# SGI-2022/Latent-Diffusion-Models-for-Shape-SDFs

Hardware: AMD Instinct MI355X
Metric: SDF queries/sec on 256^3 grid (+ DDPM sample steps/sec) (higher is better)
Workload: dtype bf16; 1 GPU; config4: decode B=64 shapes on a 256^3 grid on 1 rank (the whole grid is the one slab: no gather); batch=64, grid=256, latent_dim=256, decoder=DeepSDF 8x512 skip@4, parallelism=zslab1

## Files before the change

latent-diffusion-models-for-shape-sdfs_amd/csrc/decoder_fs.hip:

```cpp
#include "decoder_common.h"

namespace ldm {
namespace {
using namespace dec;

constexpr int kFsD = 4;
constexpr int kFsDefaultV = 2;

constexpr int kFsStep = 2048;
constexpr int kFsAct = 33 * 4 * 1024;
constexpr int kFsRed = 4 * 4 * 64 * 4;
constexpr int kFsWl = 512 * 4;
#ifndef FS_STAMP
#define FS_STAMP 0
#endif
constexpr int kFsStamp = FS_STAMP ? 128 * 8 : 0;
#ifndef FS_ABL
#define FS_ABL 0
#endif
static_assert(FS_ABL == 0 || FS_STAMP, "ablations are diagnostic builds");
constexpr int kFsLds = kFsAct + kFsRed + kFsWl + kFsStamp;
static_assert(kFsLds <= 160 * 1024, "LDS");

__host__ __device__ constexpr int fs_nparts(int S) { return S == 256 ? 15 : 16; }
__host__ __device__ constexpr int fs_nsteps(int S) { return S == 256 ? 384 : 448; }

template <typename T>
__global__ void fs_aux_pack_kernel(const float* __restrict__ beta, const float* __restrict__ wxyz,
                                   int B, T* __restrict__ aux) {
    const int id = blockIdx.x * blockDim.x + threadIdx.x;
    if (id >= B * 4 * 4 * 2 * 64) return;
    const int lane = id & 63;
    const int i = (id >> 6) & 1;
    const int slot = (id >> 7) & 3;
    const int w = (id >> 9) & 3;
    const int b = id >> 11;
    const int li = slot >> 1;
    const int p = slot & 1;
    float v[8] = {0, 0, 0, 0, 0, 0, 0, 0};
    if (lane < 32) {
        const int f = 128 * w + 64 * p + 32 * i + lane;
        const float* wx = wxyz + ((size_t)li * kHidden + f) * 3;
        const float bb = beta[((size_t)b * 2 + li) * kHidden + f];
        const float hi = Elem<T>::round(bb);
        v[0] = wx[0]; v[1] = wx[1]; v[2] = wx[2];
        v[3] = wx[0]; v[4] = wx[1]; v[5] = wx[2];
        v[6] = hi;    v[7] = bb - hi;
    }
    T* o = aux + (size_t)id * 8;
#pragma unroll
    for (int e = 0; e < 8; ++e) o[e] = (T)v[e];
}

struct FArgs {
    const uint8_t* stream;
    const uint8_t* aux;
    const float* w_last;
    const float* xyz;
    float* out;
    float b_last;
    int npts, tiles_per_shape, n_tiles;
    int N, k0;
    float vs, origin;
};

enum FsEpi { FE_NONE = 0, FE_LATE = 1, FE_EARLY = 2, FE_FIN0 = 3, FE_FIN1 = 4 };

struct FSrc {
    bool shape;
    uint32_t off;
    bool none = false;
};

template <int FV>
struct FCtx {
    int lane, wave, h;
    uint32_t voff;
    char* smem;
    __amdgpu_buffer_rsrc_t rw;
    __amdgpu_buffer_rsrc_t ra;
    uint32_t s_beg, s_end;
    uint32_t s_iss;
    uint32_t baux_w;
    uint32_t aux_w;
    uint32_t aux_next;
    u32x4 auxn[2];
    u32x4 ring[kFsD][2];
    u32x4 b[4];
    float part[4];
    float* out;
    int npts, prev_shape, prev_local;
    float b_last;
    unsigned long long* st;
    int st_i;
    bool st_on;
};

template <int FV>
__device__ __forceinline__ void stamp(FCtx<FV>& c) {
    if (FS_STAMP) {
        if (c.st_on && c.lane == 0 && c.st_i < 128) c.st[c.st_i] = __builtin_readcyclecounter();
        ++c.st_i;
    }
}

__device__ __forceinline__ u32x4 bld(__amdgpu_buffer_rsrc_t r, uint32_t voff, uint32_t soff) {
    return __builtin_bit_cast(u32x4, __builtin_amdgcn_raw_buffer_load_b128(r, voff, soff, 0));
}

template <int FV>
__device__ __forceinline__ void load_aux(FCtx<FV>& c, FSrc s) {
    if (s.none) return;
    const __amdgpu_buffer_rsrc_t r = s.shape ? c.ra : c.rw;
    c.auxn[0] = bld(r, c.voff, s.off);
    c.auxn[1] = bld(r, c.voff + 1024u, s.off);
}

__device__ __forceinline__ uint32_t opaque(uint32_t v) {
    asm volatile("" : "+v"(v));
    return v;
}

__device__ __forceinline__ int opaque_s(int v) {
    asm volatile("" : "+s"(v));
    return v;
}

template <int FV>
__device__ __forceinline__ char* lds_at(const FCtx<FV>& c, uint32_t off) {
    return c.smem + (opaque(c.voff) + off);
}
template <int FV>
__device__ __forceinline__ u32x4* act_w(const FCtx<FV>& c, int late) {
    return reinterpret_cast<u32x4*>(lds_at(c, (uint32_t)(late + 4 * c.wave) * 4096u));
}
template <int FV>
__device__ __forceinline__ const f32x4* wl_at(const FCtx<FV>& c, int p, int i) {
    const uint32_t h = opaque(c.voff) >> 9;
    return reinterpret_cast<const f32x4*>(
        c.smem + kFsAct + kFsRed + (((c.wave * 2 + p) * 2 + i) * 2) * 64 + h * 64);
}

template <int FV>
__device__ __forceinline__ float* red_w(const FCtx<FV>& c) {
    return reinterpret_cast<float*>(c.smem + kFsAct + c.wave * 4 * 64 * 4 + (opaque(c.voff) >> 2));
}

__device__ __forceinline__ void fs_bar() {
    if (FS_ABL & 4) return;
    asm volatile("s_waitcnt lgkmcnt(0)\n\ts_barrier" ::: "memory");
}

template <int FV>
__device__ __forceinline__ void read_b(FCtx<FV>& c, int pos) {
    const u32x4* p = reinterpret_cast<const u32x4*>(lds_at(c, pos * 4096));
#pragma unroll
    for (int n = 0; n < 4; ++n) c.b[n] = p[n * 64];
}

template <int FV>
__device__ __forceinline__ void issue(FCtx<FV>& c, int r) {
    const uint32_t so = c.s_iss + (uint32_t)(r >> 1) * 2u * kFsStep;
    const uint32_t vo = c.voff + (uint32_t)(r & 1) * kFsStep;
    if (FS_ABL & 1) return;
    c.ring[r][0] = bld(c.rw, vo, so);
    c.ring[r][1] = bld(c.rw, vo + 1024u, so);
}

template <int FV>
__device__ __forceinline__ void next_group(FCtx<FV>& c) {
    c.s_iss += 4u * kFsStep;
    if (c.s_iss == c.s_end) c.s_iss = c.s_beg;
}

__device__ __forceinline__ float relu_f(float x) {
    return __builtin_bit_cast(float, max(__builtin_bit_cast(int, x), 0));
}

template <typename T, int EK, int FV>
__device__ __forceinline__ void epi_unit(FCtx<FV>& c, const f32x16 (&accY)[2][4], int u) {
    const int t = u >> 1, s = u & 1;
    const int i = t >> 2, n = t & 3;
    if (FS_ABL & 2) return;
    if (EK == FE_LATE || EK == FE_EARLY) {
        u32x4 f;
#pragma unroll
        for (int q = 0; q < 4; ++q)
            f[q] = relu2(Elem<T>::pack(accY[i][n][8 * s + 2 * q], accY[i][n][8 * s + 2 * q + 1]));
        u32x4* p = act_w(c, EK == FE_LATE ? 16 : 0);
        p[((2 * i + s) * 4 + n) * 64] = f;
    } else if (EK == FE_FIN0 || EK == FE_FIN1) {
        const f32x4* w = wl_at(c, EK == FE_FIN0 ? 0 : 1, i);
        float part = c.part[n];
#pragma unroll
        for (int q = 2 * s; q < 2 * s + 2; ++q) {
            const f32x4 wv = w[q];
#pragma unroll
            for (int e = 0; e < 4; ++e) part = fmaf(relu_f(accY[i][n][4 * q + e]), wv[e], part);
        }
        c.part[n] = part;
    }
}

template <typename T, int EK, int FV>
__device__ __forceinline__ void epi_step(FCtx<FV>& c, const f32x16 (&accY)[2][4], int k) {
    if (EK == FE_NONE || k == 15) return;
    epi_unit<T, EK>(c, accY, k);
    if (k == 14) epi_unit<T, EK>(c, accY, 15);
    if (EK == FE_FIN1 && k == 14) {
        float* rw = red_w(c);
#pragma unroll
        for (int n = 0; n < 4; ++n) {
            rw[n * 64] = c.part[n];
            c.part[n] = 0.f;
        }
    }
}

template <int FV>
__device__ __forceinline__ void fin_store(const FCtx<FV>& c, int shape, int local) {
    const int lane = (int)(opaque(c.voff) >> 4);
    if (local < 0 || lane >= 32) return;
    const float* rr = reinterpret_cast<const float*>(
        c.smem + kFsAct + c.wave * 64 * 4 + (opaque(c.voff) >> 2));
    float s = 0.f;
#pragma unroll
    for (int w = 0; w < 4; ++w) s += rr[w * 4 * 64] + rr[w * 4 * 64 + 32];
    const int pt = local * kTilePoints + 32 * c.wave + lane;
    if (pt < c.npts) {
        const __amdgpu_buffer_rsrc_t ro = __builtin_amdgcn_make_buffer_rsrc(
            (void*)(c.out + (size_t)shape * c.npts), (short)0, 0x7ffffff0, 0x00020000);
        __builtin_amdgcn_raw_buffer_store_b32(__builtin_bit_cast(uint32_t, tanhf(s + c.b_last)),
                                              ro, (uint32_t)pt * 4u, 0, 2 );
    }
}

__device__ __forceinline__ void valu_slot(int v) {
    if (v == 2) __builtin_amdgcn_sched_group_barrier(0x002, 2, 0);
    else if (v == 4) __builtin_amdgcn_sched_group_barrier(0x002, 4, 0);
}

template <typename T>
__device__ __forceinline__ void mfma_pair(f32x16 (&acc)[2][4], const u32x4& a0, const u32x4& a1,
                                          const u32x4& b, int n) {
    acc[0][n] = Elem<T>::mfma(a0, b, acc[0][n]);
    acc[1][n] = Elem<T>::mfma(a1, b, acc[1][n]);
}

template <typename T, int EK, int K0, int BAR, int FV>
__device__ __forceinline__ void group4(FCtx<FV>& c, f32x16 (&acc)[2][4], const f32x16 (&accY)[2][4],
                                       int p0) {
    constexpr int BP = (FV & 1) ? 2 : 1;
    const char* gbase = (FV & 2) ? lds_at(c, (p0 + 1) * 4096) : nullptr;
#pragma unroll
    for (int r = 0; r < 4; ++r) {
        const u32x4* nb = reinterpret_cast<const u32x4*>(
            (FV & 2) ? gbase + r * 4096 : lds_at(c, (p0 + r + 1) * 4096));
        const u32x4 a0 = c.ring[r][0], a1 = c.ring[r][1];
        const int k = K0 + r;
        const int V = (EK == FE_NONE || k == 15) ? 0 : (k == 14 ? 4 : 2);
        if (r == BAR) {
#pragma unroll
            for (int n = 0; n < BP; ++n) mfma_pair<T>(acc, a0, a1, c.b[n], n);
            for (int n = 0; n < BP; ++n) {
                __builtin_amdgcn_sched_group_barrier(0x008, 2, 0);
            }
            __builtin_amdgcn_sched_barrier(0);
            fs_bar();
            __builtin_amdgcn_sched_barrier(0);
#pragma unroll
            for (int n = 0; n < BP; ++n) c.b[n] = nb[n * 64];
#pragma unroll
            for (int n = BP; n < 4; ++n) {
                mfma_pair<T>(acc, a0, a1, c.b[n], n);
                c.b[n] = nb[n * 64];
            }
            issue(c, r);
            epi_step<T, EK>(c, accY, k);
            for (int n = 0; n < BP; ++n) __builtin_amdgcn_sched_group_barrier(0x100, 1, 0);
            for (int n = BP; n < 4; ++n) {
                __builtin_amdgcn_sched_group_barrier(0x008, 1, 0);
                valu_slot(V);
                __builtin_amdgcn_sched_group_barrier(0x008, 1, 0);
                __builtin_amdgcn_sched_group_barrier(0x100, 1, 0);
                valu_slot(V);
            }
        } else {
#pragma unroll
            for (int n = 0; n < 4; ++n) {
                mfma_pair<T>(acc, a0, a1, c.b[n], n);
                c.b[n] = nb[n * 64];
            }
            issue(c, r);
            epi_step<T, EK>(c, accY, k);
#pragma unroll
            for (int n = 0; n < 4; ++n) {
                __builtin_amdgcn_sched_group_barrier(0x008, 1, 0);
                valu_slot(V);
                __builtin_amdgcn_sched_group_barrier(0x008, 1, 0);
                __builtin_amdgcn_sched_group_barrier(0x100, 1, 0);
                valu_slot(V);
            }
        }
        __builtin_amdgcn_sched_group_barrier(0x020, 2, 0);
        __builtin_amdgcn_sched_barrier(0);
    }
    next_group(c);
}

template <typename T, int EK, bool BAR, int FV>
__device__ __forceinline__ void steps16e(FCtx<FV>& c, f32x16 (&acc)[2][4],
                                         const f32x16 (&accY)[2][4], int p0) {
    group4<T, EK, 0, -1, FV>(c, acc, accY, p0);
    group4<T, EK, 4, -1, FV>(c, acc, accY, p0 + 4);
    group4<T, EK, 8, -1, FV>(c, acc, accY, p0 + 8);
    group4<T, EK, 12, BAR ? 3 : -1, FV>(c, acc, accY, p0 + 12);
}

template <typename T, int FV>
__device__ __forceinline__ void steps_plain(FCtx<FV>& c, f32x16 (&acc)[2][4],
                                            const f32x16 (&accY)[2][4], int pos0, int j0, int j1) {
#pragma unroll 1
    for (int j = j0; j < j1; j += 4) group4<T, FE_NONE, 0, -1, FV>(c, acc, accY, pos0 + j);
}

template <typename T, int EK, bool E16, int FV>
__device__ __forceinline__ void run_part(FCtx<FV>& c, f32x16 (&acc)[2][4], const f32x16 (&accY)[2][4],
                                         int nk, bool mid, bool endbar, FSrc naux, int pos0,
                                         bool bar0) {
    const f32x16 zero = {};
    const u32x4 a0 = c.auxn[0], a1 = c.auxn[1];
    if (nk == 0) {
#pragma unroll
        for (int n = 0; n < 4; ++n) {
            acc[0][n] = Elem<T>::mfma(a0, c.b[n], zero);
            acc[1][n] = Elem<T>::mfma(a1, c.b[n], zero);
        }
        load_aux(c, naux);
        stamp(c);
        return;
    }
    if (bar0) {
#pragma unroll
        for (int n = 0; n < 4; ++n) {
            acc[0][n] = Elem<T>::mfma(a0, c.b[n], zero);
            acc[1][n] = Elem<T>::mfma(a1, c.b[n], zero);
        }
        load_aux(c, naux);
        fs_bar();
        read_b(c, pos0);
    } else {
        const u32x4* p = reinterpret_cast<const u32x4*>(lds_at(c, pos0 * 4096));
#pragma unroll
        for (int n = 0; n < 4; ++n) {
            acc[0][n] = Elem<T>::mfma(a0, c.b[n], zero);
            acc[1][n] = Elem<T>::mfma(a1, c.b[n], zero);
            c.b[n] = p[n * 64];
        }
        load_aux(c, naux);
#pragma unroll
        for (int n = 0; n < 4; ++n) {
            __builtin_amdgcn_sched_group_barrier(0x008, 2, 0);
            __builtin_amdgcn_sched_group_barrier(0x100, 1, 0);
        }
        __builtin_amdgcn_sched_group_barrier(0x020, 2, 0);
        __builtin_amdgcn_sched_barrier(0);
    }
    stamp(c);
    if (!E16 && EK != FE_NONE) {
        if (mid || (endbar && nk == 16)) steps16e<T, EK, true>(c, acc, accY, pos0);
        else steps16e<T, EK, false>(c, acc, accY, pos0);
        if (EK == FE_FIN1) fin_store(c, c.prev_shape, c.prev_local);
        stamp(c);
        if (endbar && nk == 32) {
            steps_plain<T>(c, acc, accY, pos0, 16, 28);
            group4<T, FE_NONE, 0, 3, FV>(c, acc, accY, pos0 + 28);
        } else {
            steps_plain<T>(c, acc, accY, pos0, 16, nk);
        }
    } else if (E16) {
        steps_plain<T>(c, acc, accY, pos0, 0, 12);
        group4<T, FE_NONE, 0, 3, FV>(c, acc, accY, pos0 + 12);
        stamp(c);
        if (endbar) steps16e<T, EK, true>(c, acc, accY, pos0 + 16);
        else steps16e<T, EK, false>(c, acc, accY, pos0 + 16);
    } else {
        steps_plain<T>(c, acc, accY, pos0, 0, nk < 16 ? nk : 16);
        stamp(c);
        steps_plain<T>(c, acc, accY, pos0, 16, nk);
    }
    stamp(c);
}

template <typename T, bool LATE, int FV>
__device__ __forceinline__ void acc_to_lds(FCtx<FV>& c, const f32x16 (&acc)[2][4]) {
    u32x4* p = act_w(c, LATE ? 16 : 0);
#pragma unroll
    for (int i = 0; i < 2; ++i)
#pragma unroll
        for (int n = 0; n < 4; ++n) {
            u32x4 f0, f1;
            acc_to_frags<T>(acc[i][n], f0, f1);
            p[(2 * i * 4 + n) * 64] = f0;
            p[((2 * i + 1) * 4 + n) * 64] = f1;
        }
}

template <typename T, int S, bool POINTS, int FV>
__global__ __launch_bounds__(256, 1) void dec_fs_kernel(FArgs a) {
    __shared__ __attribute__((aligned(16))) char smem[kFsLds];
    FCtx<FV> c;
    c.lane = threadIdx.x & 63;
    c.wave = __builtin_amdgcn_readfirstlane(threadIdx.x >> 6);
    c.h = c.lane >> 5;
    c.voff = (uint32_t)c.lane * 16u;
    c.smem = smem;
    c.out = a.out;
    c.npts = a.npts;
    c.b_last = a.b_last;
    c.prev_shape = 0;
    c.prev_local = -1;
    c.st = reinterpret_cast<unsigned long long*>(smem + kFsAct + kFsRed + kFsWl);
    c.st_i = 0;
    c.st_on = false;
    float* wl = reinterpret_cast<float*>(smem + kFsAct + kFsRed);

    for (int i = threadIdx.x; i < 512; i += 256) wl[i] = a.w_last[i];
    __syncthreads();
    if ((int)blockIdx.x >= a.n_tiles) return;

    constexpr int NST = fs_nsteps(S);
    constexpr int NP = fs_nparts(S);
    constexpr uint32_t kFlags = 0x00020000u;
    c.rw = __builtin_amdgcn_make_buffer_rsrc((void*)a.stream, (short)0, 0x7ffffff0, kFlags);
    c.ra = __builtin_amdgcn_make_buffer_rsrc((void*)a.aux, (short)0, 0x7ffffff0, kFlags);
    c.s_beg = (uint32_t)c.wave * NST * kFsStep;
    c.s_end = c.s_beg + NST * kFsStep;
    c.s_iss = c.s_beg;
    c.baux_w = (uint32_t)(4 * NST + c.wave * NP) * kFsStep;
    auto shape_aux = [&](int tile) -> uint32_t {
        return ((uint32_t)(tile / a.tiles_per_shape) * 4u + (uint32_t)c.wave) * 4u * kFsStep;
    };
    auto bias = [&](int pi) -> FSrc { return FSrc{false, c.baux_w + (uint32_t)pi * kFsStep}; };
    auto shp = [&](int slot) -> FSrc { return FSrc{true, c.aux_w + (uint32_t)slot * kFsStep}; };
    c.aux_w = shape_aux(blockIdx.x);
#pragma unroll
    for (int r = 0; r < kFsD; ++r) issue(c, r);
    next_group(c);

    f32x16 accA[2][4], accB[2][4];
#pragma unroll
    for (int i = 0; i < 2; ++i)
#pragma unroll
        for (int n = 0; n < 4; ++n) accB[i][n] = f32x16{};
#pragma unroll
    for (int n = 0; n < 4; ++n) c.part[n] = 0.f;
#pragma unroll 1
    for (int tile = blockIdx.x; tile < a.n_tiles; tile += gridDim.x) {
        const int shape = tile / a.tiles_per_shape;
        const int local = tile - shape * a.tiles_per_shape;
        {
            const int nt = tile + (int)gridDim.x;
            c.aux_next = nt < a.n_tiles ? shape_aux(nt) : c.aux_w;
        }
        c.st_on = FS_STAMP && c.wave == 0 && tile == (int)blockIdx.x + (int)gridDim.x;
        c.st_i = 0;
        stamp(c);
        load_aux(c, shp(0));
        const uint32_t lv = opaque(c.voff);
        const bool hi = lv >= 512u;
#pragma unroll
        for (int n = 0; n < 4; ++n) {
            int pt = local * kTilePoints + 32 * n + (int)((lv >> 4) & 31u);
            if (pt >= a.npts) pt = a.npts - 1;
            float x, y, z;
            if (POINTS) {
                const float* qq = a.xyz + ((size_t)shape * a.npts + pt) * 3;
                x = qq[0];
                y = qq[1];
                z = qq[2];
            } else {
                grid_point(pt, opaque_s(a.N), a.k0, a.vs, a.origin, x, y, z);
            }
            const float xh = Elem<T>::round(x), yh = Elem<T>::round(y), zh = Elem<T>::round(z);
            u32x4 f;
            f[0] = hi ? 0u : Elem<T>::pack(xh, yh);
            f[1] = hi ? 0u : Elem<T>::pack(zh, x - xh);
            f[2] = hi ? 0u : Elem<T>::pack(y - yh, z - zh);
            f[3] = hi ? 0u : Elem<T>::pack(1.f, 1.f);
            reinterpret_cast<u32x4*>(lds_at(c, 32u * 4096u))[n * 64] = f;
        }
        read_b(c, 32);

        run_part<T, FE_NONE, false, FV>(c, accA, accB, 0, false, false, shp(1), 0, false);
        acc_to_lds<T, false, FV>(c, accA);
        stamp(c);
        run_part<T, FE_NONE, false, FV>(c, accA, accB, 0, false, false, bias(2), 0, false);
        acc_to_lds<T, true, FV>(c, accA);
        stamp(c);

        int pi = 2;
        run_part<T, FE_FIN1, false, FV>(c, accA, accB, 32, true, false, bias(pi + 1), 0, true);
        run_part<T, FE_EARLY, true, FV>(c, accB, accA, 32, true, true, bias(pi + 2), 0, false);
        pi += 2;
        constexpr int L2P = S == 256 ? 3 : 4;
#pragma unroll 1
        for (int l = 2; l < L2P; ++l, pi += 2) {
            const FSrc nx = (S == 512 && l == 3) ? shp(2) : bias(pi + 2);
            run_part<T, FE_LATE, false, FV>(c, accA, accB, 32, true, false, bias(pi + 1), 0, false);
            run_part<T, FE_EARLY, true, FV>(c, accB, accA, 32, true, true, nx, 0, false);
        }
        if (S == 256) {
            run_part<T, FE_LATE, false, FV>(c, accA, accB, 32, true, false, shp(2), 0, false);
            fs_bar();
            acc_to_lds<T, true, FV>(c, accA);
            stamp(c);
            run_part<T, FE_NONE, false, FV>(c, accA, accB, 16, false, false, shp(3), 16, true);
            run_part<T, FE_EARLY, false, FV>(c, accB, accA, 16, false, true, bias(pi + 3), 16,
                                             false);
            pi += 3;
        } else {
            run_part<T, FE_LATE, false, FV>(c, accA, accB, 32, true, false, shp(3), 0, false);
            run_part<T, FE_EARLY, true, FV>(c, accB, accA, 32, true, true, bias(pi + 2), 0, false);
            pi += 2;
        }
#pragma unroll 1
        for (int l = 5; l < 7; ++l, pi += 2) {
            run_part<T, FE_LATE, false, FV>(c, accA, accB, 32, true, false, bias(pi + 1), 0, false);
            run_part<T, FE_EARLY, true, FV>(c, accB, accA, 32, true, true, bias(pi + 2), 0, false);
        }
        run_part<T, FE_LATE, false, FV>(c, accA, accB, 32, true, false, bias(pi + 1), 0, false);
        run_part<T, FE_FIN0, false, FV>(c, accB, accA, 32, false, true, FSrc{true, 0, true}, 0,
                                        false);
        c.prev_shape = shape;
        c.prev_local = local;
        c.aux_w = c.aux_next;
    }
#pragma unroll
    for (int u = 0; u < 16; ++u) epi_unit<T, FE_FIN1>(c, accB, u);
    {
        float* rw = red_w(c);
#pragma unroll
        for (int n = 0; n < 4; ++n) rw[n * 64] = c.part[n];
    }
    fs_bar();
    fin_store(c, c.prev_shape, c.prev_local);
    asm volatile("s_waitcnt vmcnt(0)" ::: "memory");
    if (FS_STAMP && c.wave == 0) {
        __builtin_amdgcn_s_waitcnt(0);
        for (int k = c.lane; k < 128; k += 64)
            reinterpret_cast<unsigned long long*>(a.out)[(size_t)blockIdx.x * 128 + k] = c.st[k];
    }
}

template <typename T, int S, int D>
void launch_fs_d(const FArgs& a, bool points, hipStream_t s, int grid) {
    if (points)
        hipLaunchKernelGGL((dec_fs_kernel<T, S, true, D>), dim3(grid), dim3(256), 0, s, a);
    else
        hipLaunchKernelGGL((dec_fs_kernel<T, S, false, D>), dim3(grid), dim3(256), 0, s, a);
}

template <typename T, int S>
void launch_fs(const FArgs& a, bool points, hipStream_t s, int grid) {
#ifdef LDM_DEV_KNOBS
    switch (dev_knob("LDM_FS_V", kFsDefaultV)) {
        case 0: return launch_fs_d<T, S, 0>(a, points, s, grid);
        case 1: return launch_fs_d<T, S, 1>(a, points, s, grid);
        case 3: return launch_fs_d<T, S, 3>(a, points, s, grid);
        default: break;
    }
#endif
    launch_fs_d<T, S, kFsDefaultV>(a, points, s, grid);
}

}

size_t decoder_fs_aux_bytes(int B) { return (size_t)B * 4 * 4 * kFsStep; }

int decoder_fs_n_stages(int skip_width) { return fs_nsteps(skip_width == 253 ? 256 : 512); }

int decoder_fs_fwd(const ldm_decoder_t* w, const float* beta, const float* xyz, int B, int npts,
                   int N, int k0, float vs, float origin, float* out, void* ws, size_t ws_bytes,
                   hipStream_t s, int num_cus) {
    const int S = w->skip_width == 253 ? 256 : 512;
    LDM_REQUIRE(w->n_stages == fs_nsteps(S), LDM_EINVAL, "split layout: n_stages %d != %d",
                w->n_stages, fs_nsteps(S));
    LDM_REQUIRE(ws != nullptr && ws_bytes >= decoder_fs_aux_bytes(B) && LDM_ALIGNED(ws, 16),
                LDM_ENOSPC, "workspace too small: need %zu bytes, got %zu",
                decoder_fs_aux_bytes(B), ws_bytes);
    LDM_REQUIRE((size_t)B * 4 * 4 * kFsStep < 0x7ffffff0u, LDM_EINVAL,
                "split layout: %d shapes exceed the aux buffer range", B);
    {
        const int n = B * 4 * 4 * 2 * 64;
        if (w->dtype == LDM_BF16)
            hipLaunchKernelGGL(fs_aux_pack_kernel<__bf16>, dim3((n + 255) / 256), dim3(256), 0, s,
                               beta, w->wxyz, B, (__bf16*)ws);
        else
            hipLaunchKernelGGL(fs_aux_pack_kernel<_Float16>, dim3((n + 255) / 256), dim3(256), 0,
                               s, beta, w->wxyz, B, (_Float16*)ws);
        if (int e = launch_status("fs_aux_pack")) return e;
    }
    FArgs a;
    a.stream = (const uint8_t*)w->weights;
    a.aux = (const uint8_t*)ws;
    a.w_last = w->w_last;
    a.xyz = xyz;
    a.out = out;
    a.b_last = w->b_last;
    a.npts = npts;
    a.tiles_per_shape = (npts + kTilePoints - 1) / kTilePoints;
    a.n_tiles = B * a.tiles_per_shape;
    a.N = N;
    a.k0 = k0;
    a.vs = vs;
    a.origin = origin;
    const int grid = a.n_tiles < num_cus ? a.n_tiles : num_cus;
    const bool points = xyz != nullptr;
    if (w->dtype == LDM_BF16) {
        if (S == 256) launch_fs<__bf16, 256>(a, points, s, grid);
        else launch_fs<__bf16, 512>(a, points, s, grid);
    } else {
        if (S == 256) launch_fs<_Float16, 256>(a, points, s, grid);
        else launch_fs<_Float16, 512>(a, points, s, grid);
    }
    return launch_status("ldm_decoder_fwd(split)");
}

}
```

latent-diffusion-models-for-shape-sdfs_amd/csrc/decoder_common.h:

```cpp
#pragma once
#include "ldm_internal.h"

#include <math.h>

namespace ldm {
namespace dec {

#define LDM_STR2(x) #x
#define LDM_STR(x) LDM_STR2(x)

__device__ __forceinline__ float grid_axis(int i, float vs, float origin) {
#pragma clang fp contract(off)
    float t = (float)i * vs;
    return t + origin;
}

__device__ __forceinline__ void grid_point(int p, int N, int k0, float vs, float origin,
                                           float& x, float& y, float& z) {
    const int nn = N * N;
    const int k = k0 + p / nn;
    const int r = p - (p / nn) * nn;
    const int j = r / N;
    const int i = r - j * N;
    x = grid_axis(i, vs, origin);
    y = grid_axis(j, vs, origin);
    z = grid_axis(k, vs, origin);
}


template <typename T>
struct Elem;
template <>
struct Elem<__bf16> {
    static __device__ __forceinline__ unsigned pack(float a, float b) {
        typedef float f32x2 __attribute__((ext_vector_type(2)));
        const f32x2 v = {a, b};
        return __builtin_bit_cast(unsigned, __builtin_convertvector(v, bf16x2));
    }
    static __device__ __forceinline__ float round(float x) { return (float)(__bf16)x; }
    static __device__ __forceinline__ f32x16 mfma(u32x4 a, u32x4 b, f32x16 c) {
        return __builtin_amdgcn_mfma_f32_32x32x16_bf16(__builtin_bit_cast(bf16x8, a),
                                                       __builtin_bit_cast(bf16x8, b), c, 0, 0, 0);
    }
    static __device__ __forceinline__ f32x4 mfma16(u32x4 a, u32x4 b, f32x4 c) {
        return __builtin_amdgcn_mfma_f32_16x16x32_bf16(__builtin_bit_cast(bf16x8, a),
                                                       __builtin_bit_cast(bf16x8, b), c, 0, 0, 0);
    }
};
template <>
struct Elem<_Float16> {
    static __device__ __forceinline__ unsigned pack(float a, float b) {
        f16x2 v = {(_Float16)a, (_Float16)b};
        return __builtin_bit_cast(unsigned, v);
    }
    static __device__ __forceinline__ float round(float x) { return (float)(_Float16)x; }
    static __device__ __forceinline__ f32x16 mfma(u32x4 a, u32x4 b, f32x16 c) {
        return __builtin_amdgcn_mfma_f32_32x32x16_f16(__builtin_bit_cast(f16x8, a),
                                                      __builtin_bit_cast(f16x8, b), c, 0, 0, 0);
    }
    static __device__ __forceinline__ f32x4 mfma16(u32x4 a, u32x4 b, f32x4 c) {
        return __builtin_amdgcn_mfma_f32_16x16x32_f16(__builtin_bit_cast(f16x8, a),
                                                      __builtin_bit_cast(f16x8, b), c, 0, 0, 0);
    }
};


__device__ __forceinline__ unsigned relu2(unsigned v) {
    typedef short s16x2 __attribute__((ext_vector_type(2)));
    s16x2 x = __builtin_bit_cast(s16x2, v);
    const s16x2 z = {0, 0};
    x = __builtin_elementwise_max(x, z);
    return __builtin_bit_cast(unsigned, x);
}

template <typename T>
__device__ __forceinline__ void acc_to_frags(const f32x16& a, u32x4& f0, u32x4& f1) {
#pragma unroll
    for (int q = 0; q < 4; ++q) {
        f0[q] = relu2(Elem<T>::pack(a[2 * q], a[2 * q + 1]));
        f1[q] = relu2(Elem<T>::pack(a[8 + 2 * q], a[8 + 2 * q + 1]));
    }
}

}
}
```

Before: 469.1 million queries/s.

## Overlap next tile's xyz encoding and first layer with last layer's tail

Moves the computation of the next tile's input coordinates and its first layer MFMAs into the final layer part of the current tile, so the prologue of each tile overlaps the previous tile's epilogue instead of running serially at loop top. Grid-point index decomposition now uses host-precomputed magic-number division instead of integer division. The stamp instrumentation is made branch-free with a dummy slot. This adds register pressure and complexity in the loop-carried state (shape/local handoff).

```diff
diff --git a/latent-diffusion-models-for-shape-sdfs_amd/csrc/decoder_fs.hip b/latent-diffusion-models-for-shape-sdfs_amd/csrc/decoder_fs.hip
--- a/latent-diffusion-models-for-shape-sdfs_amd/csrc/decoder_fs.hip
+++ b/latent-diffusion-models-for-shape-sdfs_amd/csrc/decoder_fs.hip
@@ -14,7 +14,7 @@
 #ifndef FS_STAMP
 #define FS_STAMP 0
 #endif
-constexpr int kFsStamp = FS_STAMP ? 128 * 8 : 0;
+constexpr int kFsStamp = FS_STAMP ? 129 * 8 : 0;
 #ifndef FS_ABL
 #define FS_ABL 0
 #endif
@@ -62,14 +62,25 @@
     int npts, tiles_per_shape, n_tiles;
     int N, k0;
     float vs, origin;
+    uint32_t mN, mNN;
+    int shN, shNN;
 };
+
+inline void fs_magic(uint32_t d, uint32_t& m, int& sh) {
+    int l = 0;
+    while ((1ull << l) < d) ++l;
+    sh = 31 + l;
+    m = (uint32_t)(((1ull << sh) + d - 1) / d);
+}
+__device__ __forceinline__ int fs_div(int n, uint32_t m, int sh) {
+    return (int)(((uint64_t)(uint32_t)n * m) >> sh);
+}
 
 enum FsEpi { FE_NONE = 0, FE_LATE = 1, FE_EARLY = 2, FE_FIN0 = 3, FE_FIN1 = 4 };
 
 struct FSrc {
     bool shape;
     uint32_t off;
-    bool none = false;
 };
 
 template <int FV>
@@ -99,7 +110,7 @@
 template <int FV>
 __device__ __forceinline__ void stamp(FCtx<FV>& c) {
     if (FS_STAMP) {
-        if (c.st_on && c.lane == 0 && c.st_i < 128) c.st[c.st_i] = __builtin_readcyclecounter();
+        c.st[c.st_on && c.st_i < 128 ? c.st_i : 128] = __builtin_readcyclecounter();
         ++c.st_i;
     }
 }
@@ -110,7 +121,6 @@
 
 template <int FV>
 __device__ __forceinline__ void load_aux(FCtx<FV>& c, FSrc s) {
-    if (s.none) return;
     const __amdgpu_buffer_rsrc_t r = s.shape ? c.ra : c.rw;
     c.auxn[0] = bld(r, c.voff, s.off);
     c.auxn[1] = bld(r, c.voff + 1024u, s.off);
@@ -118,11 +128,6 @@
 
 __device__ __forceinline__ uint32_t opaque(uint32_t v) {
     asm volatile("" : "+v"(v));
-    return v;
-}
-
-__device__ __forceinline__ int opaque_s(int v) {
-    asm volatile("" : "+s"(v));
     return v;
 }
 
@@ -370,7 +375,10 @@
     if (!E16 && EK != FE_NONE) {
         if (mid || (endbar && nk == 16)) steps16e<T, EK, true>(c, acc, accY, pos0);
         else steps16e<T, EK, false>(c, acc, accY, pos0);
-        if (EK == FE_FIN1) fin_store(c, c.prev_shape, c.prev_local);
+        if (EK == FE_FIN1) {
+            stamp(c);
+            fin_store(c, c.prev_shape, c.prev_local);
+        }
         stamp(c);
         if (endbar && nk == 32) {
             steps_plain<T>(c, acc, accY, pos0, 16, 28);
@@ -404,6 +412,80 @@
             p[(2 * i * 4 + n) * 64] = f0;
             p[((2 * i + 1) * 4 + n) * 64] = f1;
         }
+}
+
+template <typename T, bool POINTS, int FV>
+__device__ __forceinline__ u32x4 xyz_frag(const FCtx<FV>& c, const FArgs& a, int shape, int local,
+                                          int n) {
+    const uint32_t lv = opaque(c.voff);
+    const bool hi = lv >= 512u;
+    int pt = local * kTilePoints + 32 * n + (int)((lv >> 4) & 31u);
+    if (pt >= a.npts) pt = a.npts - 1;
+    float x, y, z;
+    if (POINTS) {
+        const float* qq = a.xyz + ((size_t)shape * a.npts + pt) * 3;
+        x = qq[0];
+        y = qq[1];
+        z = qq[2];
+    } else {
+        const int k = fs_div(pt, a.mNN, a.shNN);
+        const int r = pt - k * (a.N * a.N);
+        const int j = fs_div(r, a.mN, a.shN);
+        x = grid_axis(r - j * a.N, a.vs, a.origin);
+        y = grid_axis(j, a.vs, a.origin);
+        z = grid_axis(a.k0 + k, a.vs, a.origin);
+    }
+    const float xh = Elem<T>::round(x), yh = Elem<T>::round(y), zh = Elem<T>::round(z);
+    u32x4 f;
+    f[0] = hi ? 0u : Elem<T>::pack(xh, yh);
+    f[1] = hi ? 0u : Elem<T>::pack(zh, x - xh);
+    f[2] = hi ? 0u : Elem<T>::pack(y - yh, z - zh);
+    f[3] = hi ? 0u : Elem<T>::pack(1.f, 1.f);
+    reinterpret_cast<u32x4*>(lds_at(c, 32u * 4096u))[n * 64] = f;
+    return f;
+}
+
+template <typename T, bool POINTS, int FV>
+__device__ __forceinline__ void run_l7p1(FCtx<FV>& c, f32x16 (&acc)[2][4], f32x16 (&accY)[2][4],
+                                         const FArgs& a, int nshape, int nlocal) {
+    const f32x16 zero = {};
+    {
+        const u32x4 a0 = c.auxn[0], a1 = c.auxn[1];
+        const u32x4* p = reinterpret_cast<const u32x4*>(lds_at(c, 0));
+#pragma unroll
+        for (int n = 0; n < 4; ++n) {
+            acc[0][n] = Elem<T>::mfma(a0, c.b[n], zero);
+            acc[1][n] = Elem<T>::mfma(a1, c.b[n], zero);
+            c.b[n] = p[n * 64];
+        }
+        load_aux(c, FSrc{true, c.aux_next});
+#pragma unroll
+        for (int n = 0; n < 4; ++n) {
+            __builtin_amdgcn_sched_group_barrier(0x008, 2, 0);
+            __builtin_amdgcn_sched_group_barrier(0x100, 1, 0);
+        }
+        __builtin_amdgcn_sched_group_barrier(0x020, 2, 0);
+        __builtin_amdgcn_sched_barrier(0);
+    }
+    stamp(c);
+    steps16e<T, FE_FIN0, true>(c, acc, accY, 0);
+    stamp(c);
+#pragma unroll
+    for (int n = 0; n < 4; ++n) {
+        const u32x4 f = xyz_frag<T, POINTS>(c, a, nshape, nlocal, n);
+        if (FS_STAMP) {
+            __builtin_amdgcn_sched_barrier(0);
+            stamp(c);
+        }
+        accY[0][n] = Elem<T>::mfma(c.auxn[0], f, zero);
+        accY[1][n] = Elem<T>::mfma(c.auxn[1], f, zero);
+        __builtin_amdgcn_sched_barrier(0);
+        stamp(c);
+    }
+    load_aux(c, FSrc{true, c.aux_next + (uint32_t)kFsStep});
+    __builtin_amdgcn_sched_barrier(0);
+    steps16e<T, FE_EARLY, true>(c, acc, accY, 16);
+    stamp(c);
 }
 
 template <typename T, int S, bool POINTS, int FV>
@@ -455,45 +537,26 @@
         for (int n = 0; n < 4; ++n) accB[i][n] = f32x16{};
 #pragma unroll
     for (int n = 0; n < 4; ++n) c.part[n] = 0.f;
+    int shape = (int)blockIdx.x / a.tiles_per_shape;
+    int local = (int)blockIdx.x - shape * a.tiles_per_shape;
+    load_aux(c, shp(0));
+#pragma unroll
+    for (int n = 0; n < 4; ++n) c.b[n] = xyz_frag<T, POINTS>(c, a, shape, local, n);
+    run_part<T, FE_NONE, false, FV>(c, accA, accB, 0, false, false, shp(1), 0, false);
+    acc_to_lds<T, false, FV>(c, accA);
 #pragma unroll 1
     for (int tile = blockIdx.x; tile < a.n_tiles; tile += gridDim.x) {
-        const int shape = tile / a.tiles_per_shape;
-        const int local = tile - shape * a.tiles_per_shape;
+        int nshape = shape, nlocal = local;
         {
             const int nt = tile + (int)gridDim.x;
-            c.aux_next = nt < a.n_tiles ? shape_aux(nt) : c.aux_w;
+            if (nt < a.n_tiles) {
+                nshape = nt / a.tiles_per_shape;
+                nlocal = nt - nshape * a.tiles_per_shape;
+            }
+            c.aux_next = ((uint32_t)nshape * 4u + (uint32_t)c.wave) * 4u * kFsStep;
         }
         c.st_on = FS_STAMP && c.wave == 0 && tile == (int)blockIdx.x + (int)gridDim.x;
         c.st_i = 0;
-        stamp(c);
-        load_aux(c, shp(0));
-        const uint32_t lv = opaque(c.voff);
-        const bool hi = lv >= 512u;
-#pragma unroll
-        for (int n = 0; n < 4; ++n) {
-            int pt = local * kTilePoints + 32 * n + (int)((lv >> 4) & 31u);
-            if (pt >= a.npts) pt = a.npts - 1;
-            float x, y, z;
-            if (POINTS) {
-                const float* qq = a.xyz + ((size_t)shape * a.npts + pt) * 3;
-                x = qq[0];
-                y = qq[1];
-                z = qq[2];
-            } else {
-                grid_point(pt, opaque_s(a.N), a.k0, a.vs, a.origin, x, y, z);
-            }
-            const float xh = Elem<T>::round(x), yh = Elem<T>::round(y), zh = Elem<T>::round(z);
-            u32x4 f;
-            f[0] = hi ? 0u : Elem<T>::pack(xh, yh);
-            f[1] = hi ? 0u : Elem<T>::pack(zh, x - xh);
-            f[2] = hi ? 0u : Elem<T>::pack(y - yh, z - zh);
-            f[3] = hi ? 0u : Elem<T>::pack(1.f, 1.f);
-            reinterpret_cast<u32x4*>(lds_at(c, 32u * 4096u))[n * 64] = f;
-        }
-        read_b(c, 32);
-
-        run_part<T, FE_NONE, false, FV>(c, accA, accB, 0, false, false, shp(1), 0, false);
-        acc_to_lds<T, false, FV>(c, accA);
         stamp(c);
         run_part<T, FE_NONE, false, FV>(c, accA, accB, 0, false, false, bias(2), 0, false);
         acc_to_lds<T, true, FV>(c, accA);
@@ -530,11 +593,12 @@
             run_part<T, FE_EARLY, true, FV>(c, accB, accA, 32, true, true, bias(pi + 2), 0, false);
         }
         run_part<T, FE_LATE, false, FV>(c, accA, accB, 32, true, false, bias(pi + 1), 0, false);
-        run_part<T, FE_FIN0, false, FV>(c, accB, accA, 32, false, true, FSrc{true, 0, true}, 0,
-                                        false);
+        run_l7p1<T, POINTS, FV>(c, accB, accA, a, nshape, nlocal);
         c.prev_shape = shape;
         c.prev_local = local;
         c.aux_w = c.aux_next;
+        shape = nshape;
+        local = nlocal;
     }
 #pragma unroll
     for (int u = 0; u < 16; ++u) epi_unit<T, FE_FIN1>(c, accB, u);
@@ -615,6 +679,13 @@
     a.k0 = k0;
     a.vs = vs;
     a.origin = origin;
+    a.mN = a.mNN = 0;
+    a.shN = a.shNN = 0;
+    if (xyz == nullptr) {
+        LDM_REQUIRE(N >= 1 && N <= 46340, LDM_EINVAL, "split layout: grid N %d out of range", N);
+        fs_magic((uint32_t)N, a.mN, a.shN);
+        fs_magic((uint32_t)N * (uint32_t)N, a.mNN, a.shNN);
+    }
     const int grid = a.n_tiles < num_cus ? a.n_tiles : num_cus;
     const bool points = xyz != nullptr;
     if (w->dtype == LDM_BF16) {
```

Result: no change. 471.6 million queries/s (median of 6 runs) (+0.5%).

## Prefetch next tile's xyz fragments and aux during last layer, use magic division

Applied to the files above, without the earlier changes.

Computes the next tile's query coordinates inside the final hidden layer's MFMA steps, writing them into a double-buffered LDS slot (activation region grows by one 4 KiB page and toggles via a_off). The next tile's aux load is also issued late inside the final pass, so the per-tile prologue (point generation, aux load, read_b) runs only for the first tile. Integer divisions for grid index decomposition are replaced with precomputed magic-multiply division. This aims to hide per-tile setup latency behind matrix work, at the cost of more registers and LDS, and an extra group4 split in steps_plain.

```diff
diff --git a/latent-diffusion-models-for-shape-sdfs_amd/csrc/decoder_common.h b/latent-diffusion-models-for-shape-sdfs_amd/csrc/decoder_common.h
--- a/latent-diffusion-models-for-shape-sdfs_amd/csrc/decoder_common.h
+++ b/latent-diffusion-models-for-shape-sdfs_amd/csrc/decoder_common.h
@@ -1,5 +1,6 @@
 #pragma once
 #include "ldm_internal.h"
+#include "magic_div.h"
 
 #include <math.h>
 
@@ -27,6 +28,17 @@
     z = grid_axis(k, vs, origin);
 }
 
+__device__ __forceinline__ void grid_point_magic(int p, int N, MagicDiv mN, MagicDiv mNN, int k0,
+                                                 float vs, float origin, float& x, float& y,
+                                                 float& z) {
+    const int kk = (int)magic_quot31((uint32_t)p, mNN.mul, mNN.shift);
+    const int r = p - kk * (N * N);
+    const int j = (int)magic_quot31((uint32_t)r, mN.mul, mN.shift);
+    const int i = r - j * N;
+    x = grid_axis(i, vs, origin);
+    y = grid_axis(j, vs, origin);
+    z = grid_axis(k0 + kk, vs, origin);
+}
 
 template <typename T>
 struct Elem;
diff --git a/latent-diffusion-models-for-shape-sdfs_amd/csrc/decoder_fs.hip b/latent-diffusion-models-for-shape-sdfs_amd/csrc/decoder_fs.hip
--- a/latent-diffusion-models-for-shape-sdfs_amd/csrc/decoder_fs.hip
+++ b/latent-diffusion-models-for-shape-sdfs_amd/csrc/decoder_fs.hip
@@ -1,4 +1,5 @@
 #include "decoder_common.h"
+#include "magic_div.h"
 
 namespace ldm {
 namespace {
@@ -8,7 +9,7 @@
 constexpr int kFsDefaultV = 2;
 
 constexpr int kFsStep = 2048;
-constexpr int kFsAct = 33 * 4 * 1024;
+constexpr int kFsAct = 34 * 4 * 1024;
 constexpr int kFsRed = 4 * 4 * 64 * 4;
 constexpr int kFsWl = 512 * 4;
 #ifndef FS_STAMP
@@ -62,14 +63,17 @@
     int npts, tiles_per_shape, n_tiles;
     int N, k0;
     float vs, origin;
+    MagicDiv mN, mNN;
 };
 
-enum FsEpi { FE_NONE = 0, FE_LATE = 1, FE_EARLY = 2, FE_FIN0 = 3, FE_FIN1 = 4 };
+enum FsEpi { FE_NONE = 0, FE_LATE = 1, FE_EARLY = 2, FE_FIN0 = 3, FE_FIN1 = 4, FE_XYZG = 5,
+             FE_XYZP = 6 };
 
 struct FSrc {
     bool shape;
     uint32_t off;
     bool none = false;
+    bool late = false;
 };
 
 template <int FV>
@@ -91,6 +95,15 @@
     float* out;
     int npts, prev_shape, prev_local;
     float b_last;
+    uint32_t a_off;
+    const float* x_row;
+    int x_pt0;
+    uint32_t x_woff;
+    int gN, gNN, gk0;
+    float gvs, gorg;
+    MagicDiv mN, mNN;
+    int xi[2];
+    float xf[6];
     unsigned long long* st;
     int st_i;
     bool st_on;
@@ -118,11 +131,6 @@
 
 __device__ __forceinline__ uint32_t opaque(uint32_t v) {
     asm volatile("" : "+v"(v));
-    return v;
-}
-
-__device__ __forceinline__ int opaque_s(int v) {
-    asm volatile("" : "+s"(v));
     return v;
 }
 
@@ -202,8 +210,52 @@
     }
 }
 
+template <typename T>
+__device__ __forceinline__ u32x4 xyz_frag(float x, float y, float z, float xh, float yh, float zh,
+                                          bool hi) {
+    u32x4 f;
+    f[0] = hi ? 0u : Elem<T>::pack(xh, yh);
+    f[1] = hi ? 0u : Elem<T>::pack(zh, x - xh);
+    f[2] = hi ? 0u : Elem<T>::pack(y - yh, z - zh);
+    f[3] = hi ? 0u : Elem<T>::pack(1.f, 1.f);
+    return f;
+}
+
+template <typename T, bool POINTS, int FV>
+__device__ __forceinline__ void xyz_step(FCtx<FV>& c, int r) {
+    if (r == 0) {
+        int pt = c.x_pt0 + (int)((c.voff >> 4) & 31u);
+        if (pt >= c.npts) pt = c.npts - 1;
+        if (POINTS) {
+            const float* qq = c.x_row + (size_t)pt * 3;
+            c.xf[0] = qq[0];
+            c.xf[1] = qq[1];
+            c.xf[2] = qq[2];
+        } else {
+            const int k = (int)magic_quot31((uint32_t)pt, c.mNN.mul, c.mNN.shift);
+            c.xi[0] = k;
+            c.xi[1] = pt - k * c.gNN;
+        }
+    } else if (r == 1) {
+        if (!POINTS) {
+            const int j = (int)magic_quot31((uint32_t)c.xi[1], c.mN.mul, c.mN.shift);
+            const int i = c.xi[1] - j * c.gN;
+            c.xf[0] = grid_axis(i, c.gvs, c.gorg);
+            c.xf[1] = grid_axis(j, c.gvs, c.gorg);
+            c.xf[2] = grid_axis(c.gk0 + c.xi[0], c.gvs, c.gorg);
+        }
+    } else if (r == 2) {
+#pragma unroll
+        for (int e = 0; e < 3; ++e) c.xf[3 + e] = Elem<T>::round(c.xf[e]);
+    } else {
+        *reinterpret_cast<u32x4*>(c.smem + (c.voff + c.x_woff)) = xyz_frag<T>(
+            c.xf[0], c.xf[1], c.xf[2], c.xf[3], c.xf[4], c.xf[5], c.voff >= 512u);
+    }
+}
+
 template <typename T, int EK, int FV>
 __device__ __forceinline__ void epi_step(FCtx<FV>& c, const f32x16 (&accY)[2][4], int k) {
+    if (EK == FE_XYZG || EK == FE_XYZP) return xyz_step<T, EK == FE_XYZP>(c, k & 3);
     if (EK == FE_NONE || k == 15) return;
     epi_unit<T, EK>(c, accY, k);
     if (k == 14) epi_unit<T, EK>(c, accY, 15);
@@ -254,11 +306,13 @@
     const char* gbase = (FV & 2) ? lds_at(c, (p0 + 1) * 4096) : nullptr;
 #pragma unroll
     for (int r = 0; r < 4; ++r) {
+        const uint32_t ao = (r == 3 && p0 + 4 == 32) ? c.a_off : 0u;
         const u32x4* nb = reinterpret_cast<const u32x4*>(
-            (FV & 2) ? gbase + r * 4096 : lds_at(c, (p0 + r + 1) * 4096));
+            (FV & 2) ? gbase + r * 4096 + ao : lds_at(c, (p0 + r + 1) * 4096 + ao));
         const u32x4 a0 = c.ring[r][0], a1 = c.ring[r][1];
         const int k = K0 + r;
-        const int V = (EK == FE_NONE || k == 15) ? 0 : (k == 14 ? 4 : 2);
+        const int V = (EK == FE_XYZG || EK == FE_XYZP) ? 2
+                      : (EK == FE_NONE || k == 15) ? 0 : (k == 14 ? 4 : 2);
         if (r == BAR) {
 #pragma unroll
             for (int n = 0; n < BP; ++n) mfma_pair<T>(acc, a0, a1, c.b[n], n);
@@ -320,11 +374,14 @@
 template <typename T, int FV>
 __device__ __forceinline__ void steps_plain(FCtx<FV>& c, f32x16 (&acc)[2][4],
                                             const f32x16 (&accY)[2][4], int pos0, int j0, int j1) {
+    const bool last = pos0 + j1 == 32 && j1 - j0 >= 4;
+    const int je = last ? j1 - 4 : j1;
 #pragma unroll 1
-    for (int j = j0; j < j1; j += 4) group4<T, FE_NONE, 0, -1, FV>(c, acc, accY, pos0 + j);
-}
-
-template <typename T, int EK, bool E16, int FV>
+    for (int j = j0; j < je; j += 4) group4<T, FE_NONE, 0, -1, FV>(c, acc, accY, pos0 + j);
+    if (last) group4<T, FE_NONE, 0, -1, FV>(c, acc, accY, pos0 + je);
+}
+
+template <typename T, int EK, bool E16, int FV, int XK = FE_NONE>
 __device__ __forceinline__ void run_part(FCtx<FV>& c, f32x16 (&acc)[2][4], const f32x16 (&accY)[2][4],
                                          int nk, bool mid, bool endbar, FSrc naux, int pos0,
                                          bool bar0) {
@@ -346,7 +403,7 @@
             acc[0][n] = Elem<T>::mfma(a0, c.b[n], zero);
             acc[1][n] = Elem<T>::mfma(a1, c.b[n], zero);
         }
-        load_aux(c, naux);
+        if (!naux.late) load_aux(c, naux);
         fs_bar();
         read_b(c, pos0);
     } else {
@@ -357,7 +414,7 @@
             acc[1][n] = Elem<T>::mfma(a1, c.b[n], zero);
             c.b[n] = p[n * 64];
         }
-        load_aux(c, naux);
+        if (!naux.late) load_aux(c, naux);
 #pragma unroll
         for (int n = 0; n < 4; ++n) {
             __builtin_amdgcn_sched_group_barrier(0x008, 2, 0);
@@ -374,7 +431,15 @@
         stamp(c);
         if (endbar && nk == 32) {
             steps_plain<T>(c, acc, accY, pos0, 16, 28);
+            if (naux.late) load_aux(c, naux);
             group4<T, FE_NONE, 0, 3, FV>(c, acc, accY, pos0 + 28);
+        } else if (XK != FE_NONE) {
+#pragma unroll 1
+            for (int j = 16; j < 32; j += 4) {
+                group4<T, XK, 0, -1, FV>(c, acc, accY, pos0 + j);
+                c.x_pt0 += 32;
+                c.x_woff += 1024u;
+            }
         } else {
             steps_plain<T>(c, acc, accY, pos0, 16, nk);
         }
@@ -420,6 +485,14 @@
     c.b_last = a.b_last;
     c.prev_shape = 0;
     c.prev_local = -1;
+    c.a_off = 0;
+    c.gN = a.N;
+    c.gNN = a.N * a.N;
+    c.gk0 = a.k0;
+    c.gvs = a.vs;
+    c.gorg = a.origin;
+    c.mN = a.mN;
+    c.mNN = a.mNN;
     c.st = reinterpret_cast<unsigned long long*>(smem + kFsAct + kFsRed + kFsWl);
     c.st_i = 0;
     c.st_on = false;
@@ -459,38 +532,45 @@
     for (int tile = blockIdx.x; tile < a.n_tiles; tile += gridDim.x) {
         const int shape = tile / a.tiles_per_shape;
         const int local = tile - shape * a.tiles_per_shape;
+        int nshape = shape, nlocal = local;
         {
             const int nt = tile + (int)gridDim.x;
-            c.aux_next = nt < a.n_tiles ? shape_aux(nt) : c.aux_w;
+            if (nt < a.n_tiles) {
+                nshape = nt / a.tiles_per_shape;
+                nlocal = nt - nshape * a.tiles_per_shape;
+            }
+            c.aux_next = ((uint32_t)nshape * 4u + (uint32_t)c.wave) * 4u * kFsStep;
         }
         c.st_on = FS_STAMP && c.wave == 0 && tile == (int)blockIdx.x + (int)gridDim.x;
         c.st_i = 0;
         stamp(c);
-        load_aux(c, shp(0));
-        const uint32_t lv = opaque(c.voff);
-        const bool hi = lv >= 512u;
-#pragma unroll
-        for (int n = 0; n < 4; ++n) {
-            int pt = local * kTilePoints + 32 * n + (int)((lv >> 4) & 31u);
-            if (pt >= a.npts) pt = a.npts - 1;
-            float x, y, z;
-            if (POINTS) {
-                const float* qq = a.xyz + ((size_t)shape * a.npts + pt) * 3;
-                x = qq[0];
-                y = qq[1];
-                z = qq[2];
-            } else {
-                grid_point(pt, opaque_s(a.N), a.k0, a.vs, a.origin, x, y, z);
+        if (tile == (int)blockIdx.x) {
+            load_aux(c, shp(0));
+            const uint32_t lv = opaque(c.voff);
+            const bool hi = lv >= 512u;
+#pragma unroll
+            for (int n = 0; n < 4; ++n) {
+                int pt = local * kTilePoints + 32 * n + (int)((lv >> 4) & 31u);
+                if (pt >= a.npts) pt = a.npts - 1;
+                float x, y, z;
+                if (POINTS) {
+                    const float* qq = a.xyz + ((size_t)shape * a.npts + pt) * 3;
+                    x = qq[0];
+                    y = qq[1];
+                    z = qq[2];
+                } else {
+                    grid_point_magic(pt, a.N, a.mN, a.mNN, a.k0, a.vs, a.origin, x, y, z);
+                }
+                const float xh = Elem<T>::round(x), yh = Elem<T>::round(y),
+                            zh = Elem<T>::round(z);
+                reinterpret_cast<u32x4*>(lds_at(c, 32u * 4096u))[n * 64] =
+                    xyz_frag<T>(x, y, z, xh, yh, zh, hi);
             }
-            const float xh = Elem<T>::round(x), yh = Elem<T>::round(y), zh = Elem<T>::round(z);
-            u32x4 f;
-            f[0] = hi ? 0u : Elem<T>::pack(xh, yh);
-            f[1] = hi ? 0u : Elem<T>::pack(zh, x - xh);
-            f[2] = hi ? 0u : Elem<T>::pack(y - yh, z - zh);
-            f[3] = hi ? 0u : Elem<T>::pack(1.f, 1.f);
-            reinterpret_cast<u32x4*>(lds_at(c, 32u * 4096u))[n * 64] = f;
-        }
-        read_b(c, 32);
+            read_b(c, 32);
+        }
+        c.x_pt0 = nlocal * kTilePoints;
+        c.x_woff = 32u * 4096u + (c.a_off ^ 4096u);
+        if (POINTS) c.x_row = a.xyz + (size_t)nshape * a.npts * 3;
 
         run_part<T, FE_NONE, false, FV>(c, accA, accB, 0, false, false, shp(1), 0, false);
         acc_to_lds<T, false, FV>(c, accA);
@@ -529,9 +609,11 @@
             run_part<T, FE_LATE, false, FV>(c, accA, accB, 32, true, false, bias(pi + 1), 0, false);
             run_part<T, FE_EARLY, true, FV>(c, accB, accA, 32, true, true, bias(pi + 2), 0, false);
         }
-        run_part<T, FE_LATE, false, FV>(c, accA, accB, 32, true, false, bias(pi + 1), 0, false);
-        run_part<T, FE_FIN0, false, FV>(c, accB, accA, 32, false, true, FSrc{true, 0, true}, 0,
-                                        false);
+        run_part<T, FE_LATE, false, FV, POINTS ? FE_XYZP : FE_XYZG>(
+            c, accA, accB, 32, true, false, bias(pi + 1), 0, false);
+        c.a_off ^= 4096u;
+        run_part<T, FE_FIN0, false, FV>(c, accB, accA, 32, false, true,
+                                        FSrc{true, c.aux_next, false, true}, 0, false);
         c.prev_shape = shape;
         c.prev_local = local;
         c.aux_w = c.aux_next;
@@ -615,6 +697,8 @@
     a.k0 = k0;
     a.vs = vs;
     a.origin = origin;
+    a.mN = magic_div31((uint32_t)(N > 0 ? N : 1));
+    a.mNN = magic_div31((uint32_t)(N > 0 ? N * N : 1));
     const int grid = a.n_tiles < num_cus ? a.n_tiles : num_cus;
     const bool points = xyz != nullptr;
     if (w->dtype == LDM_BF16) {
diff --git a/latent-diffusion-models-for-shape-sdfs_amd/csrc/magic_div.h b/latent-diffusion-models-for-shape-sdfs_amd/csrc/magic_div.h
--- /dev/null
+++ b/latent-diffusion-models-for-shape-sdfs_amd/csrc/magic_div.h
@@ -0,0 +1,31 @@
+#pragma once
+#include <stdint.h>
+
+#if defined(__HIPCC__)
+#define LDM_MAGIC_HD __host__ __device__
+#else
+#define LDM_MAGIC_HD
+#endif
+
+namespace ldm {
+
+struct MagicDiv {
+    uint32_t mul;
+    uint32_t shift;
+};
+
+LDM_MAGIC_HD inline MagicDiv magic_div31(uint32_t d) {
+    uint32_t l = 0;
+    while (l < 31 && (1u << l) < d) ++l;
+    const uint64_t p = 1ull << (31 + l);
+    MagicDiv m;
+    m.mul = (uint32_t)((p + d - 1) / d);
+    m.shift = l;
+    return m;
+}
+
+LDM_MAGIC_HD inline uint32_t magic_quot31(uint32_t n, uint32_t mul, uint32_t shift) {
+    return (uint32_t)(((uint64_t)(n << 1) * mul) >> 32) >> shift;
+}
+
+}
```

Result: no change. 465.6 million queries/s before, 466.5 million queries/s after, median of 6 (+0.2%).
